# selbouhaddani/PPLS

Measured on AMD Instinct MI355X. Metric: EM iterations/sec + log-lik rel-err vs CPU ref, n=1e6 p=q=2000 r=5, higher is better.
Workload: dtype f64

## Files before the change

### include/ppls_debug.h

```cpp
#ifndef PPLS_AMD_PPLS_DEBUG_H
#define PPLS_AMD_PPLS_DEBUG_H

#include "ppls.h"

#ifdef __cplusplus
extern "C" {
#endif

int ppls_sweep_timing(ppls_ctx* ctx, double* total_ms, int64_t* launches, int reset);
int ppls_sweep_balance(ppls_ctx* ctx, double* w8, int64_t* bounds, int cap, int* n_bounds);
int ppls_comm_info(ppls_ctx* ctx, int* nranks, int* rank, double* allreduce_ms, int64_t* allreduce_calls,
                   int reset);
int ppls_xprod_info(ppls_ctx* ctx, int r, int* ready, int64_t* bytes_per_pass, double* flops, int* rows_per_wave);
int ppls_xprod_setup_times(ppls_ctx* ctx, double* gram_ms, double* allreduce_ms, double* total_ms);
int ppls_xprod_tile_timing(ppls_ctx* ctx, int reps, double* ms);
int ppls_xprod_stats(ppls_ctx* ctx, const ppls_theta* th, int r, double* stats);
int ppls_sweep_stats(ppls_ctx* ctx, const ppls_theta* th, int r, int want_mu, double* stats, double* mu);
int ppls_finalize_stats(ppls_ctx* ctx, const ppls_theta* th, int r, int type, int iter, const double* stats,
                        const double* gram_cur, const double* vstate_in, const double* xpM, int ldx, int ldy,
                        double* W_next, double* C_next, double* scalars, ppls_expect* mom, double* loglik,
                        double* gram_nxt, double* vstate_out, double* gram_stats, int* status3);
int ppls_finalize_plan(ppls_ctx* ctx, int r, int type, int* templated, int* KX, int* KY, int* staged,
                       int64_t* stage_budget);
int ppls_sweep_info(ppls_ctx* ctx, int r, int64_t* bytes_per_sweep, int* variant, int* grid);
int ppls_sweep_kernel(ppls_ctx* ctx, int r, char* buf, int len);
int ppls_gram_int8(ppls_ctx* ctx, int which, double* G, int* nmod, int* L, double* ms);
int ppls_gram_shifts(ppls_ctx* ctx, int* shift, int P, int* count);
int ppls_oz_residue_host(double x, int shift, int l, int* r);
int ppls_oz_crt_host(const int* r, int nmod, double* out);
int ppls_oz_modulus(int l);
int ppls_gram_info(ppls_ctx* ctx, int* int8_used, int* nmod, int* L, double* ms);
int ppls_meta_info(ppls_ctx* ctx, int* path);
int ppls_meta_xprod_info(ppls_ctx* ctx, int* npop, int64_t* formations, double* form_ms);
int ppls_xprod_meta_stats(ppls_ctx* ctx, const double* W, const double* C, const double* params, double* stats);
int ppls_xprod_meta_timing(ppls_ctx* ctx, int reps, double* ms);
int ppls_xprod_meta_nt(int K, int P);
int ppls_rank1_mu_coefficients(const double* params5, double* coef4);
int ppls_gram(ppls_ctx* ctx, int xory, int nsplit, double* G, double* ms);
int ppls_gram_weighted(ppls_ctx* ctx, int xory, int nsplit, const int32_t* count, double* G, double* ms);
int ppls_xgram_permuted(ppls_ctx* ctx, int nsplit, const int64_t* perm, double* C , double* ms);
int ppls_xperm_occupancy(int f32);
int ppls_xperm_timing(ppls_ctx* ctx, double* ms4);
int ppls_gram_occupancy(int f32);
int ppls_gram_occupancy_weighted(int f32);
int ppls_spd_inverse(ppls_ctx* ctx, const double* A, int p, int a, int method, double* out, int* info, double* ms);
int ppls_philox4x32_10(ppls_ctx* ctx, const uint32_t* ctr, int64_t count, uint64_t key, uint32_t* out);

#define PPLS_FTRACE_LEN 48
int ppls_finalize_trace(ppls_ctx* ctx, int64_t* stamps, double* tick_ns);
#define PPLS_STRACE_MAX_WG 4096
int ppls_sweep_trace(ppls_ctx* ctx, int64_t* stamps, int cap, int* n, double* tick_ns);
int ppls_cv_timing(ppls_ctx* ctx, double* out6, int reset);

int ppls_xprod_get(ppls_ctx* ctx, double* S, int* P, int* ldx);
// ... 20 lines not shown
```

### ppls_amd/_lib.py

```python
from __future__ import annotations

import ctypes as ct
import os

import numpy as np

_HERE = os.path.dirname(os.path.abspath(__file__))
LIB_PATH = os.path.join(_HERE, "libppls_amd.so")

PPLS_OK = 0
PPLS_ORTH_SVD = 0
PPLS_ORTH_QR = 1
PPLS_LAYOUT_COLMAJOR = 0
PPLS_LAYOUT_ROWMAJOR = 1

_dp = ct.POINTER(ct.c_double)


class PplsTheta(ct.Structure):
    _fields_ = [("W", _dp), ("C", _dp), ("B", _dp), ("sigT", _dp),
                ("sigE", ct.c_double), ("sigF", ct.c_double), ("sigH", ct.c_double)]


class PplsExpect(ct.Structure):
# ... 86 lines not shown
    "ppls_finalize_stats": (ct.c_int, [ct.c_void_p, ct.POINTER(PplsTheta), ct.c_int, ct.c_int, ct.c_int, _dp, _dp, _dp,
                                       _dp, ct.c_int, ct.c_int, _dp, _dp, _dp, ct.POINTER(PplsExpect), _dp, _dp,
                                       _dp, _dp, ct.POINTER(ct.c_int)]),
    "ppls_finalize_plan": (ct.c_int, [ct.c_void_p, ct.c_int, ct.c_int, ct.POINTER(ct.c_int), ct.POINTER(ct.c_int),
                                      ct.POINTER(ct.c_int), ct.POINTER(ct.c_int), ct.POINTER(ct.c_int64)]),
    "ppls_xprod_info": (ct.c_int, [ct.c_void_p, ct.c_int, ct.POINTER(ct.c_int), ct.POINTER(ct.c_int64), _dp,
                                   ct.POINTER(ct.c_int)]),
    "ppls_sweep_timing": (ct.c_int, [ct.c_void_p, _dp, ct.POINTER(ct.c_int64), ct.c_int]),
    "ppls_sweep_balance": (ct.c_int, [ct.c_void_p, _dp, ct.POINTER(ct.c_int64), ct.c_int, ct.POINTER(ct.c_int)]),
    "ppls_comm_info": (ct.c_int, [ct.c_void_p, ct.POINTER(ct.c_int), ct.POINTER(ct.c_int), _dp,
                                  ct.POINTER(ct.c_int64), ct.c_int]),
    "ppls_finalize_trace": (ct.c_int, [ct.c_void_p, ct.POINTER(ct.c_int64), _dp]),
    "ppls_sweep_trace": (ct.c_int, [ct.c_void_p, ct.POINTER(ct.c_int64), ct.c_int, ct.POINTER(ct.c_int), _dp]),
    "ppls_sweep_info": (ct.c_int, [ct.c_void_p, ct.c_int, ct.POINTER(ct.c_int64), ct.POINTER(ct.c_int),
                                   ct.POINTER(ct.c_int)]),
    "ppls_sweep_kernel": (ct.c_int, [ct.c_void_p, ct.c_int, ct.c_char_p, ct.c_int]),
    "ppls_meta_info": (ct.c_int, [ct.c_void_p, ct.POINTER(ct.c_int)]),
    "ppls_gram_int8": (ct.c_int, [ct.c_void_p, ct.c_int, _dp, ct.POINTER(ct.c_int), ct.POINTER(ct.c_int), _dp]),
    "ppls_oz_residue_host": (ct.c_int, [ct.c_double, ct.c_int, ct.c_int, ct.POINTER(ct.c_int)]),
    "ppls_oz_crt_host": (ct.c_int, [ct.POINTER(ct.c_int), ct.c_int, _dp]),
    "ppls_oz_modulus": (ct.c_int, [ct.c_int]),
    "ppls_gram_info": (ct.c_int, [ct.c_void_p, ct.POINTER(ct.c_int), ct.POINTER(ct.c_int), ct.POINTER(ct.c_int),
                                  _dp]),
    "ppls_gram_shifts": (ct.c_int, [ct.c_void_p, ct.POINTER(ct.c_int), ct.c_int, ct.POINTER(ct.c_int)]),
    "ppls_finalize_host": (ct.c_int, [_dp, _dp, _dp, ct.c_double, ct.c_double, ct.c_double, ct.c_int,
                                      ct.c_int, ct.c_int, ct.POINTER(PplsTheta), ct.c_int,
                                      ct.POINTER(PplsTheta), ct.POINTER(PplsExpect), _dp]),
    "ppls_mu_coefficients": (ct.c_int, [ct.POINTER(PplsTheta), ct.c_int, _dp]),
    "ppls_set_data_from": (ct.c_int, [ct.c_void_p, ct.c_void_p, _i64p, ct.c_int64, ct.c_int64]),
    "ppls_xprod_downdate": (ct.c_int, [ct.c_void_p, ct.c_void_p, _i64p, ct.c_int64]),
    "ppls_xprod_resample": (ct.c_int, [ct.c_void_p, ct.c_void_p, ct.POINTER(ct.c_int32)]),
    "ppls_xprod_permute": (ct.c_int, [ct.c_void_p, ct.c_void_p, _i64p]),
    "ppls_xgram_permuted": (ct.c_int, [ct.c_void_p, ct.c_int, _i64p, _dp, _dp]),
    "ppls_xperm_occupancy": (ct.c_int, [ct.c_int]),
    "ppls_xperm_timing": (ct.c_int, [ct.c_void_p, _dp]),
    "ppls_predict": (ct.c_int, [ct.c_void_p, _dp, _dp, _dp, ct.c_int, ct.c_int, _dp, ct.c_int64, ct.c_int, _dp]),
    "ppls_heldout_sse": (ct.c_int, [ct.c_void_p, _dp, _dp, _dp, ct.c_int, _i64p, ct.c_int64, _dp]),
    "ppls_cv_ppls": (ct.c_int, [ct.c_void_p, ct.c_int, ct.c_int, ct.POINTER(ct.c_int32), _i64p, ct.c_int,
                                ct.c_double, ct.c_int, ct.POINTER(PplsTheta), _dp, ct.POINTER(ct.c_int)]),
    "ppls_cv_timing": (ct.c_int, [ct.c_void_p, _dp, ct.c_int]),
    "ppls_scale_data": (ct.c_int, [ct.c_void_p, ct.c_int, ct.c_int]),
    "ppls_get_scaling": (ct.c_int, [ct.c_void_p, _dp, _dp]),
    "ppls_scale_timing": (ct.c_int, [ct.c_void_p, _dp, _dp]),
    "ppls_xprod_get": (ct.c_int, [ct.c_void_p, _dp, ct.POINTER(ct.c_int), ct.POINTER(ct.c_int)]),
    "ppls_stream_begin":(ct.c_int, [ct.c_void_p, ct.c_int, ct.c_int, ct.c_int, ct.c_int]),
    "ppls_stream_rows": (ct.c_int, [ct.c_void_p, _dp, _dp, ct.c_int64, ct.c_int]),
# ... 131 lines not shown
```

### ppls_amd/api.py

```python
from __future__ import annotations

import ctypes as ct
import itertools
import math
import time
import warnings

import numpy as np

from . import _lib
from ._lib import Expect, PplsError, Theta, dptr


def pop_rows(pop_sizes, row0, n_local):
    sizes = np.asarray(pop_sizes, dtype=np.int64)
    ends = np.cumsum(sizes)
    begins = ends - sizes
    lo, hi = int(row0), int(row0) + int(n_local)
    local = np.clip(np.minimum(ends, hi) - np.maximum(begins, lo), 0, None).astype(np.int64)
    return np.ascontiguousarray(local), np.ascontiguousarray(sizes)


class Context:

# ... 529 lines not shown
        return G, ms.value

    def gram_occupancy(self, f32=False, weighted=False):
        fn = self._L.ppls_gram_occupancy_weighted if weighted else self._L.ppls_gram_occupancy
        return int(fn(int(bool(f32))))

    def gram_int8(self, which=2, want=True):
        P = self.p if which == 0 else self.q if which == 1 else int(round(np.sqrt(self.xprod_info()["bytes_per_pass"] / 8)))
        G = np.zeros((P, P), order="F") if want else None
        nm, L, ms = ct.c_int(), ct.c_int(), np.zeros(4)
        self._chk(self._L.ppls_gram_int8(self.h, int(which), dptr(G), ct.byref(nm), ct.byref(L), dptr(ms)))
        return G, dict(nmod=nm.value, L=L.value, ms=ms.tolist(), shift=self.gram_shifts())

    def gram_shifts(self):
        k = ct.c_int()
        self._chk(self._L.ppls_gram_shifts(self.h, None, 0, ct.byref(k)))
        out = (ct.c_int * max(k.value, 1))()
        self._chk(self._L.ppls_gram_shifts(self.h, out, k.value, ct.byref(k)))
        return np.array(out[:k.value], dtype=np.int64)

    def gram_info(self):
        u, nm, L, ms = ct.c_int(), ct.c_int(), ct.c_int(), np.zeros(4)
        self._chk(self._L.ppls_gram_info(self.h, ct.byref(u), ct.byref(nm), ct.byref(L), dptr(ms)))
        return dict(int8=bool(u.value), nmod=nm.value, L=L.value, ms=ms.tolist())

    def spd_inverse(self, A, method=1):
        A = np.asarray(A, dtype=np.float64)
        one = A.ndim == 2
        A3 = A[None] if one else A
        a, p = A3.shape[0], A3.shape[1]
        Af = np.ascontiguousarray(np.transpose(A3, (0, 2, 1)))
        out = np.empty_like(Af)
        info = (ct.c_int * a)()
        ms = ct.c_double()
        self._chk(self._L.ppls_spd_inverse(self.h, dptr(Af), int(p), int(a), int(method), dptr(out), info,
                                            ct.byref(ms)))
        inv = np.transpose(out, (0, 2, 1))
        return (inv[0] if one else inv), np.array(list(info)), ms.value

    def xprod_prepare(self):
        ms, tot = ct.c_double(), ct.c_double()
        self._chk(self._L.ppls_xprod_prepare(self.h, ct.byref(ms), ct.byref(tot)))
        return ms.value, tot.value

    def xprod_release(self):
        self._chk(self._L.ppls_xprod_release(self.h))
        self._stream_folds = None
# ... 1384 lines not shown
```

### ppls_amd/csrc/ppls_capi.cpp

```cpp
#include <hip/hip_runtime.h>
#include <rccl/rccl.h>
#include <rocblas/rocblas.h>
#include <rocsolver/rocsolver.h>

#include <algorithm>
#include <atomic>
#include <chrono>
#include <cmath>
#include <cstdarg>
#include <cstdio>
#include <cstring>
#include <functional>
#include <string>
#include <utility>
#include <vector>

#include "../../include/ppls.h"
#include "../../include/ppls_debug.h"
#include "ppls_kernels.h"
#include "ppls_math.h"
#include "ppls_cv.h"
#include "ppls_o2m.h"
#include "ppls_permute.h"
#include "ppls_scale.h"
// ... 59 lines not shown
  int* status = nullptr;
  long long* ftrace = nullptr;
  unsigned* team_bar = nullptr;
  double* team_part = nullptr;
  long long* strace = nullptr;
  int balance = 0;
  bool bal_done = false;
  int64_t bal_n = -1;
  int bal_grid = -1;
  double bal_w[8] = {1, 1, 1, 1, 1, 1, 1, 1};
  int64_t* bal_bounds = nullptr;
  double* coefs = nullptr;
  double* scratch = nullptr;
  size_t scratch_bytes = 0;
  int* stop_d = nullptr;
  int* stop_mirror = nullptr;
  int* stop_mirror_dev = nullptr;
  const int* sweep_stop = nullptr;
  double stop_atol = 0.0;
  int em_r = 0, em_cur = 0, em_iter = 0;
  bool em_active = false;
  int xprod = 0;
  int xprod_rw = 0;
  int gram_int8 = 0;
  int oz_used = 0, oz_nmod = 0, oz_L = 0;
  std::vector<int> oz_shift;
  double oz_ms[4] = {0, 0, 0, 0};
  int8_t* oz_planes = nullptr;
  uint8_t* oz_res = nullptr;
  size_t oz_planes_len = 0, oz_res_len = 0;
  bool xp_ready = false;
  bool xp_active = false;
  bool xp_pending_gram = false;
  int xprod_fuse = 1;
  bool xp_explicit = false;
  int meta_path = 0;
  int meta_xprod = 0;
  double* mx_S = nullptr;
  int mx_K = 0;
  std::vector<int64_t> mx_local, mx_total;
  int64_t mx_formations = 0;
  double mx_form_ms = 0.0;
  int meta_device = 1;
  int vorth = 8;
  double* xp_S = nullptr;
  double* xp_M = nullptr;
  double xp_setup_ms = 0.0;
  double xp_setup_total_ms = 0.0;
  double xp_setup_ar_ms = 0.0;
  int xp_nsplit = 0;
  int* gram_q = nullptr;
  int64_t gq_key[8] = {-1, -1, -1, -1, -1, -1, -1, -1};
  rocblas_handle blas = nullptr;
// ... 81 lines not shown
    if (e_ != hipSuccess)                                                                 \
      return fail((c), PPLS_E_HIP, "%s: %s (%s:%d)", #call, hipGetErrorString(e_), __FILE__, \
                  __LINE__);                                                              \
  } while (0)

#define RCCLCHK(c, call)                                                                  \
  do {                                                                                    \
    ncclResult_t e_ = (call);                                                             \
    if (e_ != ncclSuccess)                                                                \
      return fail((c), PPLS_E_COMM, "%s: %s", #call, ncclGetErrorString(e_));            \
  } while (0)

void oz_free(ppls_ctx* c);
bool oz_held(const ppls_ctx* c);

template <typename T>
int dalloc(ppls_ctx* c, T** p, size_t count) {
  if (*p) {
    (void)hipFree(*p);
    *p = nullptr;
  }
  if (count == 0) count = 1;
  hipError_t e = hipMalloc((void**)p, count * sizeof(T));
  if (e == hipErrorOutOfMemory && oz_held(c) && (void*)p != (void*)&c->oz_planes && (void*)p != (void*)&c->oz_res) {
    (void)hipGetLastError();
    (void)hipStreamSynchronize(c->stream);
    oz_free(c);
    e = hipMalloc((void**)p, count * sizeof(T));
  }
  if (e != hipSuccess) {
    *p = nullptr;
    return fail(c, PPLS_E_NOMEM, "hipMalloc(%zu bytes): %s", count * sizeof(T), hipGetErrorString(e));
  }
  return PPLS_OK;
}

template <typename T>
void dfree(T*& p) {
  if (p) (void)hipFree(p);
  p = nullptr;
}

int ld_of(int p, int f32 = 0, int pad = 1) {
  const int es = f32 ? 4 : 8;
  const long bytes = (long)p * es;
  if (!pad || bytes < 1024 || (!f32 && p <= 2048)) return f32 ? (p + 3) & ~3 : (p + 1) & ~1;
  const long al = bytes >= 16384 ? 4096 : 128;
// ... 494 lines not shown
  if (!part_in && (rc = dalloc(c, &part, (size_t)ppls_gram_part_doubles(g.p, nsplit)))) return rc;
  if ((rc = gram_queue(c, g, n, req, &q))) { if (!part_in) dfree(part); return rc; }
  hipEvent_t e0 = nullptr, e1 = nullptr;
  hipError_t e = hipSuccess;
  if (ms) {
    e = hipEventCreate(&e0);
    if (e == hipSuccess) e = hipEventCreate(&e1);
    if (e == hipSuccess) e = hipEventRecord(e0, c->stream);
  }
  if (e == hipSuccess)
    e = ppls_launch_gram_joint(g.X, g.ldx, g.xcols, g.xreal, g.Y, g.ldy, g.ycols, g.yreal, c->dtype, n, g.p, nsplit, part,
                               q, cnt, c->stream);
  if (e == hipSuccess && ms) e = hipEventRecord(e1, c->stream);
  if (e == hipSuccess) e = ppls_launch_gram_finish(part, nsplit, g.p, g.xreal, g.xcols, g.yreal, G, c->stream);
  if (e == hipSuccess) e = hipStreamSynchronize(c->stream);
  if (e == hipSuccess && ms) e = hipEventElapsedTime(ms, e0, e1);
  if (e0) (void)hipEventDestroy(e0);
  if (e1) (void)hipEventDestroy(e1);
  if (!part_in) dfree(part);
  if (e != hipSuccess) return fail(c, PPLS_E_HIP, "MFMA Gram: %s", hipGetErrorString(e));
  return PPLS_OK;
}

bool oz_held(const ppls_ctx* c) { return c->oz_planes || c->oz_res; }

void oz_free(ppls_ctx* c) {
  dfree(c->oz_planes);
  dfree(c->oz_res);
  c->oz_planes = nullptr;
  c->oz_res = nullptr;
  c->oz_planes_len = c->oz_res_len = 0;
}

int gram_run_oz(ppls_ctx* c, const GramShape& g, int64_t n, double* G, float* ms) {
  const int P = g.p, Pp = (P + 255) / 256 * 256;
  const int64_t nkb = (n + PPLS_OZ_KS - 1) / PPLS_OZ_KS;
  const int dtype = c->dtype;
  struct Bufs {
    double* part = nullptr;
    double* st = nullptr;
    int* shift = nullptr;
    hipEvent_t ev[5] = {nullptr, nullptr, nullptr, nullptr, nullptr};
    ~Bufs() {
      dfree(part); dfree(st); dfree(shift);
      for (auto e : ev) if (e) (void)hipEventDestroy(e);
    }
  } b;
  int rc;
  const int chunks = (int)std::max<int64_t>(1, std::min<int64_t>(256, n / 2048));
  if ((rc = dalloc(c, &b.part, (size_t)chunks * 2 * Pp)) || (rc = dalloc(c, &b.st, (size_t)2 * Pp)) ||
      (rc = dalloc(c, &b.shift, (size_t)Pp)))
    return rc;
  for (auto& e : b.ev) HIPCHK(c, hipEventCreate(&e));
  HIPCHK(c, hipEventRecord(b.ev[0], c->stream));
// ... 8 lines not shown
  double qmax = 0.0;
  for (int j = 0; j < P; ++j) {
    if (!live(j) || !(st[(size_t)j] > 0.0)) continue;
    int ex = 0;
    (void)std::frexp(st[(size_t)j], &ex);
    const double cj = std::max(1.0, std::ldexp(1.0, ex) * std::sqrt((double)n / st[(size_t)Pp + j]));
    const int Lj = 53 + (int)std::ceil(std::log2(cj)) + 2;
    L = std::max(L, Lj);
    shift[(size_t)j] = Lj - ex;
    const double q = std::ldexp(std::sqrt(st[(size_t)Pp + j]), Lj - ex) + 0.5 * std::sqrt((double)n);
    qmax = std::max(qmax, q * q);
  }
  c->oz_L = L;
  c->oz_shift.assign(shift.begin(), shift.begin() + P);
  if (L > 62) return 1;
  const double need = std::log2(std::max(qmax, 1.0)) + 1.0 + 1e-7;
  double bits = 0.0;
  int nmod = 0;
  while (nmod < PPLS_OZ_MAXMOD && bits < need) bits += std::log2((double)ppls_oz_modulus(nmod++));
  if (bits < need) return 1;
  nmod = std::max(nmod, 12);
  c->oz_nmod = nmod;
  const int T = Pp / 256, ntiles = T * (T + 1) / 2, nsplit = ppls_oz_splits(nkb);
  const int64_t pstride = nkb * Pp * PPLS_OZ_KS;
  const size_t need_planes = (size_t)nmod * pstride, need_res = (size_t)nmod * nsplit * ntiles * 65536;
  if (need_planes > c->oz_planes_len || need_res > c->oz_res_len) {
    HIPCHK(c, hipStreamSynchronize(c->stream));
    oz_free(c);
    size_t fr = 0, tot = 0;
    if (hipMemGetInfo(&fr, &tot) != hipSuccess) return 1;
    const double want = (double)need_planes + (double)need_res;
    if (want > (double)fr - std::max(1073741824.0, 0.05 * (double)fr)) return 1;
    if (dalloc(c, &c->oz_planes, need_planes) || dalloc(c, &c->oz_res, need_res)) {
      c->err.clear();
      oz_free(c);
      return 1;
    }
    c->oz_planes_len = need_planes;
    c->oz_res_len = need_res;
  }
  int8_t* planes = c->oz_planes;
  uint8_t* res = c->oz_res;
  HIPCHK(c, hipMemcpyAsync(b.shift, shift.data(), sizeof(int) * Pp, hipMemcpyHostToDevice, c->stream));
  HIPCHK(c, ppls_launch_oz_residues(g.X, g.ldx, g.xcols, g.xreal, g.Y, g.ldy, g.yreal, dtype, Pp, n, nkb, b.shift,
                                    nmod, planes, pstride, c->stream));
  HIPCHK(c, hipEventRecord(b.ev[1], c->stream));
  HIPCHK(c, ppls_launch_oz_syrk(planes, pstride, Pp, nkb, nmod, res, c->stream));
  HIPCHK(c, hipEventRecord(b.ev[2], c->stream));
  HIPCHK(c, ppls_launch_oz_finish(res, nmod, nsplit, Pp, g.xcols, g.xreal, g.yreal, P, b.shift, G, c->stream));
  HIPCHK(c, hipEventRecord(b.ev[3], c->stream));
  HIPCHK(c, hipStreamSynchronize(c->stream));
  float t01 = 0.f, t12 = 0.f, t23 = 0.f, t03 = 0.f;
  HIPCHK(c, hipEventElapsedTime(&t01, b.ev[0], b.ev[1]));
  HIPCHK(c, hipEventElapsedTime(&t12, b.ev[1], b.ev[2]));
  HIPCHK(c, hipEventElapsedTime(&t23, b.ev[2], b.ev[3]));
  HIPCHK(c, hipEventElapsedTime(&t03, b.ev[0], b.ev[3]));
  c->oz_ms[0] = t01;
  c->oz_ms[1] = t12;
  c->oz_ms[2] = t23;
  c->oz_ms[3] = t03;
  if (ms) *ms = t03;
  return PPLS_OK;
}

int gram_run_s(ppls_ctx* c, const GramShape& g, int64_t n, double* G, float* ms, double* part) {
  c->oz_used = 0;
  if (c->gram_int8) {
    const int rc = gram_run_oz(c, g, n, G, ms);
    if (rc == PPLS_OK) {
      c->oz_used = 1;
      return PPLS_OK;
    }
    if (rc < 0) return rc;
  }
  return gram_run(c, g, n, 0, G, ms, part);
}

int xprod_setup(ppls_ctx* c);
bool xprod_choose(ppls_ctx* c, int max_steps, int r);

int64_t xprod_rows(const ppls_ctx* c) { return (c->n_total + c->nranks - 1) / c->nranks; }

double xprod_bytes(ppls_ctx* c) {
  const GramShape g = gram_shape(c, true, 0);
  const double PP = (double)g.p * g.p;
  return 8.0 * PP + 8.0 * (double)ppls_gram_part_doubles(g.p, gram_nsplit(c, g, xprod_rows(c), 0)) +
         16.0 * g.p * PPLS_RMAX;
}

int xprod_begin(ppls_ctx* c, int steps, int r) {
// ... 49 lines not shown
  }
  const auto ta = std::chrono::steady_clock::now();
  if ((rc = allreduce(c, c->xp_S, PP))) return rc;
  HIPCHK(c, hipStreamSynchronize(c->stream));
  c->xp_setup_ar_ms = collective(c) ? std::chrono::duration<double, std::milli>(std::chrono::steady_clock::now() - ta).count() : 0.0;
  c->xp_setup_total_ms = std::chrono::duration<double, std::milli>(std::chrono::steady_clock::now() - t0).count();
  c->xp_ready = true;
  c->xp_serial = ++g_xp_serial;
  return PPLS_OK;
}

bool xprod_choose(ppls_ctx* c, int max_steps, int r) {
  if (c->st_state == 2) return true;
  if (c->xprod == 0) return false;
  if (c->xprod == 1) return true;
  if (!c->xp_ready && xprod_bytes(c) > c->mem_free_min - std::max(1073741824.0, 0.05 * c->mem_free_min))
    return false;
  const double P = (double)(c->ldx + c->ldy);
  const double n = (double)((c->n_total + c->nranks - 1) / c->nranks);
  const double esz = c->dtype ? 4.0 : 8.0;
  const bool split = c->sweep_mode != 3 && !c->dtype && ppls_split_supported(r, c->ldx, c->ldy) > 0;
  const double t_sweep = (split ? 1.0 : 2.0) * esz * n * P / 6.5e12 + 5e-6;
  const double t_pass = 8.0 * P * P / 6.5e12 + 5e-6;
  const double gram_rate = c->gram_int8 ? 1.0e14 : 55e12;
  const double t_setup = c->xp_ready ? 0.0 : n * P * P / gram_rate + (c->nranks > 1 ? 16.0 * P * P / 100e9 : 0.0);
  return ((double)max_steps + 1.0) * (t_sweep - t_pass) > t_setup;
}

int xprod_stats(ppls_ctx* c, int r, int slot, bool fuse) {
  int rc;
  const int P = c->ldx + c->ldy;
  if (!c->xp_ready && (rc = xprod_setup(c))) return rc;
  if (!c->xp_M) {
    if ((rc = dalloc(c, &c->xp_M, (size_t)P * 2 * PPLS_RMAX))) return rc;
  }
  hipEvent_t e0, e1;
  if ((rc = timing_pair(c, &e0, &e1))) return rc;
  if (e0) HIPCHK(c, hipEventRecord(e0, c->stream));
  const int rw = ppls_xprod_tile_rows(P, r, c->xprod_rw, c->num_cus);
  const bool defer = fuse && c->xprod_fuse && r <= 8 && P <= 6144;
  HIPCHK(c, ppls_launch_xprod_tile(c->xp_S, c->ldx, c->ldy, r, rw, c->W[slot], c->C[slot], c->sc[slot], c->stats,
                                   c->xp_M, c->sweep_stop, defer ? 0 : 1, c->stream));
  c->xp_pending_gram = defer;
  if (e1) HIPCHK(c, hipEventRecord(e1, c->stream));
  return PPLS_OK;
}

// ... 407 lines not shown
    c->xprod = (int)value;
    if (value == 0 && was != 0 && !c->xp_explicit && c->st_state == 0) {
      HIPCHK(c, hipStreamSynchronize(c->stream));
      xprod_free(c);
    }
  } else if (!strcmp(key, "meta_device")) {
    c->meta_device = value ? 1 : 0;
  } else if (!strcmp(key, "meta_xprod")) {
    if (value != 0 && value != 1) return fail(c, PPLS_E_ARG, "meta_xprod must be 0 (sweep the rows) or 1 (population cross-products)");
    c->meta_xprod = (int)value;
    if (!c->meta_xprod && c->mx_S) {
      HIPCHK(c, hipStreamSynchronize(c->stream));
      meta_xp_free(c);
    }
  } else if (!strcmp(key, "vorth")) {
    if (value < 1 || value > 255) return fail(c, PPLS_E_ARG, "vorth must be in [1, 255]");
    c->vorth = (int)value;
  } else if (!strcmp(key, "xprod_fuse")) {
    c->xprod_fuse = value ? 1 : 0;
  } else if (!strcmp(key, "var_chol")) {
    if (value < 0 || value > 2) return fail(c, PPLS_E_ARG, "var_chol must be 0 (LU), 1 (Cholesky) or 2 (rocSOLVER Cholesky)");
    c->var_chol = (int)value;
  } else if (!strcmp(key, "gram_int8")) {
    if (value < 0 || value > 1) return fail(c, PPLS_E_ARG, "gram_int8 must be 0 (fp64 MFMA Gram) or 1 (int8 CRT form)");
    if ((int)value != c->gram_int8) {
      c->gram_int8 = (int)value;
      if (c->xp_ready && !c->xp_explicit) {
        dfree(c->xp_S);
        c->xp_ready = false;
      }
      if (!c->gram_int8) {
        HIPCHK(c, hipStreamSynchronize(c->stream));
        oz_free(c);
      }
    }
  } else if (!strcmp(key, "xprod_rw")) {
    if (value != 0 && value != 1 && value != 2 && value != 4 && value != 8)
      return fail(c, PPLS_E_ARG, "xprod_rw must be 0, 1, 2, 4 or 8");
    c->xprod_rw = (int)value;
  } else if (!strcmp(key, "o2m_path")) {
    if (value < 0 || value > 2) return fail(c, PPLS_E_ARG, "o2m_path must be 0 (auto), 1 (fused) or 2 (two-phase)");
    c->o2m_path = (int)value;
  } else if (!strcmp(key, "timing")) {
    if (value < 0) return fail(c, PPLS_E_ARG, "timing must be >= 0");
    c->timing = (int)value;
    c->sweep_count = 0;
  } else {
    return fail(c, PPLS_E_ARG, "unknown option '%s'", key);
  }
  return PPLS_OK;
}

void ppls_shard_range(int64_t n_total, int nranks, int rank, int64_t* row0, int64_t* n_local) {
  if (nranks < 1) nranks = 1;
  const int64_t b = n_total * rank / nranks, e = n_total * (rank + 1) / nranks;
  if (row0) *row0 = b;
  if (n_local) *n_local = e - b;
}
// ... 2849 lines not shown
    rc = fail(c, PPLS_E_HIP, "int8 gram: copy-out failed");
  dfree(dG);
  if (!rc && ms) for (int k = 0; k < 4; ++k) ms[k] = c->oz_ms[k];
  return rc;
}

int ppls_gram_shifts(ppls_ctx* c, int* shift, int P, int* count) {
  if (!c) return PPLS_E_ARG;
  const int k = (int)c->oz_shift.size();
  if (count) *count = k;
  if (shift) for (int j = 0; j < std::min(P, k); ++j) shift[j] = c->oz_shift[(size_t)j];
  return PPLS_OK;
}

int ppls_gram_info(ppls_ctx* c, int* int8_used, int* nmod, int* L, double* ms) {
  if (!c) return PPLS_E_ARG;
  if (int8_used) *int8_used = c->oz_used;
  if (nmod) *nmod = c->oz_nmod;
  if (L) *L = c->oz_L;
  if (ms) for (int k = 0; k < 4; ++k) ms[k] = c->oz_ms[k];
  return PPLS_OK;
}

int ppls_meta_info(ppls_ctx* c, int* path) {
  if (!c || !path) return PPLS_E_ARG;
  *path = c->meta_path;
  return PPLS_OK;
}

int ppls_sweep_kernel(ppls_ctx* c, int r, char* buf, int len) {
  if (!c || !buf || len < 1) return PPLS_E_ARG;
  if (r < 1 || r > PPLS_RMAX) return fail(c, PPLS_E_ARG, "bad r");
  PplsSweepArgs a;
  const int plan = sweep_plan(c, r, &a);
  const int nt = c->nt_loads > 0 ||
                 (c->nt_loads < 0 && 8.0 * sweep_rows(c) * (double)(c->ldx + c->ldy) > 256.0 * (1 << 20));
  char k[128];
  if (plan == 3) {
    if (ppls_split_describe(&a, k, sizeof k) != 0) return fail(c, PPLS_E_STATE, "no split instantiation for r=%d", r);
  } else {
    const bool rows64 = c->dots_rows ? c->dots_rows == 64 : sweep_rows(c) >= 32768;
    const int64_t wtiles = (sweep_rows(c) + (rows64 ? 63 : 31)) / (rows64 ? 64 : 32);
    const bool pair = c->dots_pair >= 0 ? c->dots_pair == 1 : wtiles < (int64_t)c->num_cus * 4 * (rows64 ? 2 : 3);
    snprintf(k, sizeof k, "panel<%s,%d> (mfmadots %d rows/%s + acc, %d chunks)", c->dtype ? "float" : "double", r,
             rows64 ? 64 : 32, pair ? "wave pair" : "wave", a.grid);
  }
// ... 395 lines not shown
  std::vector<std::vector<int64_t>> in_fold((size_t)nfolds);
  for (int64_t i = 0; i < c->n_local; ++i) {
    if (fold_of_row[i] < 0 || fold_of_row[i] >= nfolds) return fail(c, PPLS_E_ARG, "fold_of_row[%lld]=%d outside [0,%d)", (long long)i, fold_of_row[i], nfolds);
    in_fold[(size_t)fold_of_row[i]].push_back(i);
  }
  for (int f = 0; f < nfolds; ++f)
    if ((int64_t)in_fold[(size_t)f].size() > fold_total[f])
      return fail(c, PPLS_E_ARG, "fold %d: %zu local rows, %lld over all ranks", f, in_fold[(size_t)f].size(), (long long)fold_total[f]);
  for (int k = 0; !o2m && k < nfolds * a; ++k)
    if (!init[k].W || !init[k].C || !init[k].B || !init[k].sigT) return fail(c, PPLS_E_ARG, "init[%d] has NULL fields", k);
  HIPCHK(c, hipSetDevice(c->device));
  int rc;
  if (!c->cv_train && (rc = ppls_ctx_create(c->device, &c->cv_train))) return fail(c, rc, "could not create the training context");
  ppls_ctx* t = c->cv_train;
  t->xprod = c->xprod;
  t->xprod_rw = c->xprod_rw;
  t->xprod_fuse = c->xprod_fuse;
  t->o2m_path = c->o2m_path;
  if (t->gram_int8 && !c->gram_int8) {
    HIPCHK(c, hipStreamSynchronize(t->stream));
    oz_free(t);
  }
  t->gram_int8 = c->gram_int8;
  t->ldpad = c->ldpad;
  t->sweep_mode = c->sweep_mode;
  t->grid_opt = c->grid_opt;
  t->nt_loads = c->nt_loads;
  t->reducer = c->reducer;
  t->reducer_user = c->reducer_user;
  t->comm = c->comm;
  t->nranks = c->nranks;
  t->rank = c->rank;
  const int p = c->p, q = c->q;
  std::vector<double> W((size_t)p * a), C((size_t)q * a), B((size_t)a), sig((size_t)4 * a), sse((size_t)a);
  std::vector<int64_t> train;
  for (int f = 0; f < nfolds; ++f) {
    const std::vector<int64_t>& out = in_fold[(size_t)f];
    train.clear();
    for (int64_t i = 0; i < c->n_local; ++i)
      if (fold_of_row[i] != f) train.push_back(i);
    const int64_t n_train = c->n_total - fold_total[f];
    if (n_train < 1) return fail(c, PPLS_E_ARG, "fold %d leaves no training row", f);
    if ((rc = ppls_set_data_from(t, c, train.data(), (int64_t)train.size(), n_train))) { c->err = t->err; return rc; }
    if ((o2m || xprod_choose(t, a * max_steps, 1)) && fold_total[f] <= n_train)
      if ((rc = ppls_xprod_downdate(t, c, out.data(), (int64_t)out.size()))) { c->err = t->err; return rc; }
    ppls_seq_fit fit;
// ... 1455 lines not shown
```

### ppls_amd/csrc/ppls_kernels.h

```cpp
#pragma once

#include <hip/hip_runtime.h>
#include <stdint.h>

#include "ppls_math.h"

#define PPLS_SWEEP_SLOTS 4
#define PPLS_FUSED_RMAX 8

struct PplsSweepArgs {
  const double* X;
  const double* Y;
  int64_t n_local;
  int p, q;
  int ldx, ldy;
  const double* Wp;
  const double* Cp;
  const PplsScalars* sc;
  double* part;
  int64_t part_ld;
  double* mu;
  int write_mu;
  int r;
  int ns;
// ... 70 lines not shown
  const double* Cp;
  int m;
  PplsRank1* st;
  double* tw;
  double* tc;
  const double* consW;
  const double* consC;
  PplsRank1 cons_val;
  int cons_mask;
  double* Wdst;
  double* Cdst;
  PplsScalars* scdst;
  double* lv;
  double* Gkeep;
  int step, max_steps, crit_abs;
  double atol;
  int* stop;
  int* stop_mirror;
};

#define PPLS_META_KMAX 1024
#define PPLS_OZ_MAXMOD 20
#define PPLS_OZ_KS 64
struct PplsMetaStepArgs {
  const double* stats;
  int64_t part_ld;
  int K, p, q, ldx, ldy;
  const double* N;
  const double* ssq;
  PplsRank1* st;
  PplsScalars* sc;
  double* W;
  double* C;
  double* log;
  int64_t log_ld;
  int step, max_steps, crit_abs;
  double atol;
  int* stop;
  int* stop_mirror;
  double ssqX, ssqY, Ntot;
};

extern "C" {
hipError_t ppls_launch_meta_step(const PplsMetaStepArgs* a, hipStream_t st);
int ppls_split_supported(int r, int ldx, int ldy);
hipError_t ppls_launch_sweep_split(const PplsSweepArgs* a, hipStream_t st);
// ... 43 lines not shown
hipError_t ppls_launch_xtmu(const void* X, int f32, int64_t n, int ld, const double* mu, int a, int chunks,
                            double* part, int64_t part_ld, hipStream_t st);
hipError_t ppls_launch_varmat(const double* G, const double* cxt, const double* w, int p, double ctt, double k1,
                              double k2, double bstar, double s4, double N, double* M, double* sst_exp,
                              double* sst_star, hipStream_t st);
hipError_t ppls_launch_negdiag(double* M, int p, double* se, hipStream_t st);
hipError_t ppls_launch_negate(double* M, int64_t len, hipStream_t st);
hipError_t ppls_launch_symdiag(double* M, int p, double* se, hipStream_t st);
int64_t ppls_spd_inverse_work(int p, int a);
hipError_t ppls_spd_inverse_batched(double* A, int p, int a, double* work, int* info, hipStream_t st);
hipError_t ppls_launch_to_colmajor(const double* src, int64_t n, int p, int ld, double* dst,
                                   hipStream_t st);
int ppls_oz_modulus(int l);
hipError_t ppls_launch_oz_colstats(const void* X, int ldx, int xcols, int xreal, const void* Y, int ldy, int yreal,
                                   int f32, int Pp, int64_t n, int chunks, double* part, double* out, hipStream_t st);
hipError_t ppls_launch_oz_residues(const void* X, int ldx, int xcols, int xreal, const void* Y, int ldy, int yreal,
                                   int f32, int Pp, int64_t n, int64_t nkb, const int* shift, int nmod, int8_t* planes,
                                   int64_t pstride, hipStream_t st);
int ppls_oz_splits(int64_t nkb);
hipError_t ppls_launch_oz_syrk(const int8_t* planes, int64_t pstride, int Pp, int64_t nkb, int nmod, uint8_t* part,
                               hipStream_t st);
hipError_t ppls_launch_oz_finish(const uint8_t* part, int nmod, int nsplit, int Pp, int xcols, int xreal, int yreal,
                                 int P, const int* shift, double* G, hipStream_t st);
}
```

### ppls_amd/csrc/ppls_ozaki.hip

```cpp
#include <hip/hip_runtime.h>
#include <stdint.h>

#include <type_traits>

#include "ppls_device.h"
#include "ppls_kernels.h"

namespace {

constexpr int OZ_TT = 256;
constexpr int OZ_KS = PPLS_OZ_KS;
constexpr int OZ_PANEL = OZ_TT * OZ_KS;
constexpr int OZ_SPLIT_STAGES = 1024;

__host__ __device__ constexpr int oz_mod(int l) {
  switch (l) {
    case 0: return 256;  case 1: return 255;  case 2: return 253;  case 3: return 251;  case 4: return 247;
    case 5: return 241;  case 6: return 239;  case 7: return 233;  case 8: return 229;  case 9: return 227;
    case 10: return 223; case 11: return 217; case 12: return 211; case 13: return 199; case 14: return 197;
    case 15: return 193; case 16: return 191; case 17: return 181; case 18: return 179; case 19: return 173;
    default: return 1;
  }
}

// ... 244 lines not shown
    for (int j = 0; j < NJ; ++j)
#pragma unroll
      for (int r = 0; r < 16; ++r) {
        const int v = acc[i][j][r] % m;
        acc[i][j][r] = v < 0 ? v + m : v;
      }
  if (idle) return;
  uint8_t* o = out + (int64_t)it * OZ_TT * OZ_TT;
#pragma unroll
  for (int i = 0; i < 4; ++i)
#pragma unroll
    for (int j = 0; j < NJ; ++j) {
      const int col = CT * wj + 32 * j + (lane & 31);
#pragma unroll
      for (int gq = 0; gq < 4; ++gq) {
        const int row = 128 * wi + 32 * i + 8 * gq + 4 * h;
        const uint32_t v = (uint32_t)acc[i][j][4 * gq] | ((uint32_t)acc[i][j][4 * gq + 1] << 8) |
                           ((uint32_t)acc[i][j][4 * gq + 2] << 16) | ((uint32_t)acc[i][j][4 * gq + 3] << 24);
        *(uint32_t*)(o + (int64_t)col * OZ_TT + row) = v;
      }
    }
}

namespace {

template <int NMOD>
__host__ __device__ __forceinline__ double oz_crt(const int (&r)[NMOD], const OzTab& tab) {
  int d[NMOD];
#pragma unroll
  for (int l = 0; l < NMOD; ++l) {
    const int m = oz_mod(l);
    int t = r[l];
#pragma unroll
    for (int k = 0; k < l; ++k) {
      t = t - d[k] + 2 * m;
      t = (t * tab.inv[l][k]) % m;
    }
    d[l] = t;
  }
  uint32_t v[6] = {(uint32_t)d[NMOD - 1], 0, 0, 0, 0, 0};
#pragma unroll
  for (int l = NMOD - 2; l >= 0; --l) {
    uint64_t carry = (uint64_t)d[l];
#pragma unroll
    for (int q = 0; q < 6; ++q) {
      const uint64_t x = (uint64_t)v[q] * (uint64_t)oz_mod(l) + carry;
// ... 162 lines not shown
  const int64_t grid = (items + 7) / 8 * 8;
  if (grid > 0x7fffffff) return hipErrorInvalidValue;
#define OZ_SYRK(AV)                                                                                             \
  case AV:                                                                                                      \
    hipLaunchKernelGGL(ppls_oz_syrk_kernel<AV>, dim3((unsigned)grid), dim3(((AV) & 4) ? 512 : 256), 0, st, planes, \
                       pstride, Pp, nkb, nmod, nsplit, ntiles, part);                                           \
    break;
  switch (variant) {
    OZ_SYRK(0)
#ifdef OZ_LAB
    OZ_SYRK(1) OZ_SYRK(2) OZ_SYRK(4) OZ_SYRK(5) OZ_SYRK(6)
#endif
    default: return hipErrorInvalidValue;
  }
#undef OZ_SYRK
  return hipGetLastError();
}

hipError_t ppls_launch_oz_syrk(const int8_t* planes, int64_t pstride, int Pp, int64_t nkb, int nmod, uint8_t* part,
                               hipStream_t st) {
  return ppls_launch_oz_syrk_v(0, planes, pstride, Pp, nkb, nmod, part, st);
}

hipError_t ppls_launch_oz_finish(const uint8_t* part, int nmod, int nsplit, int Pp, int xcols, int xreal, int yreal,
                                 int P, const int* shift, double* G, hipStream_t st) {
  const OzCols g{xreal, xcols, yreal};
  const int T = Pp / OZ_TT, ntiles = T * (T + 1) / 2;
  const dim3 grid((unsigned)ntiles, (unsigned)(OZ_TT / 16));
#define OZ_FIN(N)                                                                                               \
  case N:                                                                                                       \
    hipLaunchKernelGGL((ppls_oz_finish_kernel<N>), grid, dim3(256), 0, st, part, nsplit, ntiles, g, P, shift, G); \
    break;
  switch (nmod) {
    OZ_NMOD_CASES(OZ_FIN)
    default: return hipErrorInvalidValue;
  }
#undef OZ_FIN
  return hipGetLastError();
}

}
```

Baseline: 207.9.

## Auto-enable int8 Ozaki Gram by size and process rows in bounded groups

The int8 CRT (Ozaki) Gram path now defaults to an auto mode that switches on when rows·P² is large, which covers this workload's size. The single large residue-plane and partial-result buffers are replaced by one workspace sized by a planner. The planner splits the rows into groups that fit a fraction of HBM, runs residues and syrk per group, and folds partial residues modulo each prime into an accumulator before the final CRT. This is meant to replace the fp64 MFMA Gram with integer matrix ops while bounding memory, at the cost of an extra fold kernel per group and a per-call memory query. The change of default also alters the cost model that decides whether the cross-product path is used.

```diff
diff --git a/include/ppls_debug.h b/include/ppls_debug.h
--- a/include/ppls_debug.h
+++ b/include/ppls_debug.h
@@ -30,6 +30,10 @@
 int ppls_oz_crt_host(const int* r, int nmod, double* out);
 int ppls_oz_modulus(int l);
 int ppls_gram_info(ppls_ctx* ctx, int* int8_used, int* nmod, int* L, double* ms);
+int64_t ppls_oz_plan_groups(int64_t n, int Pp, int nmod, int num_cus, int64_t total_hbm, int64_t free_hbm,
+                            int force_group, int* G);
+int ppls_gram_int8_plan(ppls_ctx* ctx, int* group, int64_t* ws_bytes);
+int ppls_gram_int8_auto(int64_t n_total, int nranks, int P);
 int ppls_meta_info(ppls_ctx* ctx, int* path);
 int ppls_meta_xprod_info(ppls_ctx* ctx, int* npop, int64_t* formations, double* form_ms);
 int ppls_xprod_meta_stats(ppls_ctx* ctx, const double* W, const double* C, const double* params, double* stats);
diff --git a/ppls_amd/_lib.py b/ppls_amd/_lib.py
--- a/ppls_amd/_lib.py
+++ b/ppls_amd/_lib.py
@@ -132,6 +132,10 @@
     "ppls_oz_modulus": (ct.c_int, [ct.c_int]),
     "ppls_gram_info": (ct.c_int, [ct.c_void_p, ct.POINTER(ct.c_int), ct.POINTER(ct.c_int), ct.POINTER(ct.c_int),
                                   _dp]),
+    "ppls_oz_plan_groups": (ct.c_int64, [ct.c_int64, ct.c_int, ct.c_int, ct.c_int, ct.c_int64, ct.c_int64, ct.c_int,
+                                         ct.POINTER(ct.c_int)]),
+    "ppls_gram_int8_plan": (ct.c_int, [ct.c_void_p, ct.POINTER(ct.c_int), ct.POINTER(ct.c_int64)]),
+    "ppls_gram_int8_auto": (ct.c_int, [ct.c_int64, ct.c_int, ct.c_int]),
     "ppls_gram_shifts": (ct.c_int, [ct.c_void_p, ct.POINTER(ct.c_int), ct.c_int, ct.POINTER(ct.c_int)]),
     "ppls_finalize_host": (ct.c_int, [_dp, _dp, _dp, ct.c_double, ct.c_double, ct.c_double, ct.c_int,
                                       ct.c_int, ct.c_int, ct.POINTER(PplsTheta), ct.c_int,
diff --git a/ppls_amd/api.py b/ppls_amd/api.py
--- a/ppls_amd/api.py
+++ b/ppls_amd/api.py
@@ -575,7 +575,9 @@
     def gram_info(self):
         u, nm, L, ms = ct.c_int(), ct.c_int(), ct.c_int(), np.zeros(4)
         self._chk(self._L.ppls_gram_info(self.h, ct.byref(u), ct.byref(nm), ct.byref(L), dptr(ms)))
-        return dict(int8=bool(u.value), nmod=nm.value, L=L.value, ms=ms.tolist())
+        G, ws = ct.c_int(), ct.c_int64()
+        self._chk(self._L.ppls_gram_int8_plan(self.h, ct.byref(G), ct.byref(ws)))
+        return dict(int8=bool(u.value), nmod=nm.value, L=L.value, ms=ms.tolist(), group=G.value, ws_bytes=ws.value)
 
     def spd_inverse(self, A, method=1):
         A = np.asarray(A, dtype=np.float64)
diff --git a/ppls_amd/csrc/ppls_capi.cpp b/ppls_amd/csrc/ppls_capi.cpp
--- a/ppls_amd/csrc/ppls_capi.cpp
+++ b/ppls_amd/csrc/ppls_capi.cpp
@@ -105,13 +105,14 @@
   bool em_active = false;
   int xprod = 0;
   int xprod_rw = 0;
-  int gram_int8 = 0;
+  int gram_int8 = -1;
+  int oz_group = 0;
   int oz_used = 0, oz_nmod = 0, oz_L = 0;
+  int oz_G = 0;
   std::vector<int> oz_shift;
   double oz_ms[4] = {0, 0, 0, 0};
-  int8_t* oz_planes = nullptr;
-  uint8_t* oz_res = nullptr;
-  size_t oz_planes_len = 0, oz_res_len = 0;
+  uint8_t* oz_ws = nullptr;
+  size_t oz_ws_len = 0;
   bool xp_ready = false;
   bool xp_active = false;
   bool xp_pending_gram = false;
@@ -239,7 +240,7 @@
   }
   if (count == 0) count = 1;
   hipError_t e = hipMalloc((void**)p, count * sizeof(T));
-  if (e == hipErrorOutOfMemory && oz_held(c) && (void*)p != (void*)&c->oz_planes && (void*)p != (void*)&c->oz_res) {
+  if (e == hipErrorOutOfMemory && oz_held(c) && (void*)p != (void*)&c->oz_ws) {
     (void)hipGetLastError();
     (void)hipStreamSynchronize(c->stream);
     oz_free(c);
@@ -780,14 +781,15 @@
   return PPLS_OK;
 }
 
-bool oz_held(const ppls_ctx* c) { return c->oz_planes || c->oz_res; }
+bool oz_held(const ppls_ctx* c) { return c->oz_ws != nullptr; }
 
 void oz_free(ppls_ctx* c) {
-  dfree(c->oz_planes);
-  dfree(c->oz_res);
-  c->oz_planes = nullptr;
-  c->oz_res = nullptr;
-  c->oz_planes_len = c->oz_res_len = 0;
+  dfree(c->oz_ws);
+  c->oz_ws_len = 0;
+}
+
+bool gram_wants_int8(const ppls_ctx* c, int P) {
+  return c->gram_int8 == 1 || (c->gram_int8 < 0 && ppls_gram_int8_auto(c->n_total, c->nranks, P));
 }
 
 int gram_run_oz(ppls_ctx* c, const GramShape& g, int64_t n, double* G, float* ms) {
@@ -842,41 +844,67 @@
   nmod = std::max(nmod, 12);
   c->oz_nmod = nmod;
   const int T = Pp / 256, ntiles = T * (T + 1) / 2, nsplit = ppls_oz_splits(nkb);
-  const int64_t pstride = nkb * Pp * PPLS_OZ_KS;
-  const size_t need_planes = (size_t)nmod * pstride, need_res = (size_t)nmod * nsplit * ntiles * 65536;
-  if (need_planes > c->oz_planes_len || need_res > c->oz_res_len) {
+  size_t fr = 0, tot = 0;
+  if (hipMemGetInfo(&fr, &tot) != hipSuccess) return 1;
+  int Gs = 0;
+  const int64_t ws_need = ppls_oz_plan_groups(n, Pp, nmod, c->num_cus, (int64_t)tot, (int64_t)(fr + c->oz_ws_len),
+                                           c->oz_group, &Gs);
+  if (ws_need <= 0) return 1;
+  if ((size_t)ws_need > c->oz_ws_len) {
     HIPCHK(c, hipStreamSynchronize(c->stream));
     oz_free(c);
-    size_t fr = 0, tot = 0;
-    if (hipMemGetInfo(&fr, &tot) != hipSuccess) return 1;
-    const double want = (double)need_planes + (double)need_res;
-    if (want > (double)fr - std::max(1073741824.0, 0.05 * (double)fr)) return 1;
-    if (dalloc(c, &c->oz_planes, need_planes) || dalloc(c, &c->oz_res, need_res)) {
+    if (dalloc(c, &c->oz_ws, (size_t)ws_need)) {
       c->err.clear();
       oz_free(c);
       return 1;
     }
-    c->oz_planes_len = need_planes;
-    c->oz_res_len = need_res;
-  }
-  int8_t* planes = c->oz_planes;
-  uint8_t* res = c->oz_res;
+    c->oz_ws_len = (size_t)ws_need;
+  }
+  c->oz_G = Gs;
+  const int ngroups = (nsplit + Gs - 1) / Gs;
+  const int64_t gstages = std::min<int64_t>((int64_t)Gs * 1024, nkb), grows = (int64_t)Gs * 65536;
+  const size_t plane_bytes = (size_t)nmod * gstages * Pp * PPLS_OZ_KS;
+  int8_t* planes = (int8_t*)c->oz_ws;
+  uint8_t* res = c->oz_ws + plane_bytes;
+  uint8_t* acc = res + (size_t)nmod * Gs * ntiles * 65536;
+  struct GroupEvents {
+    std::vector<hipEvent_t> v;
+    ~GroupEvents() { for (auto e : v) if (e) (void)hipEventDestroy(e); }
+  } ge;
+  ge.v.assign((size_t)2 * ngroups, nullptr);
+  for (auto& e : ge.v) HIPCHK(c, hipEventCreate(&e));
   HIPCHK(c, hipMemcpyAsync(b.shift, shift.data(), sizeof(int) * Pp, hipMemcpyHostToDevice, c->stream));
-  HIPCHK(c, ppls_launch_oz_residues(g.X, g.ldx, g.xcols, g.xreal, g.Y, g.ldy, g.yreal, dtype, Pp, n, nkb, b.shift,
-                                    nmod, planes, pstride, c->stream));
-  HIPCHK(c, hipEventRecord(b.ev[1], c->stream));
-  HIPCHK(c, ppls_launch_oz_syrk(planes, pstride, Pp, nkb, nmod, res, c->stream));
+  const size_t esz = dtype ? 4 : 8;
+  for (int k = 0; k < ngroups; ++k) {
+    const int64_t row0 = (int64_t)k * grows, rows = std::min<int64_t>(grows, n - row0);
+    const int64_t nkb_k = (rows + PPLS_OZ_KS - 1) / PPLS_OZ_KS, pstride = nkb_k * Pp * PPLS_OZ_KS;
+    const void* Xk = (const char*)g.X + (size_t)row0 * g.ldx * esz;
+    const void* Yk = g.Y ? (const void*)((const char*)g.Y + (size_t)row0 * g.ldy * esz) : nullptr;
+    HIPCHK(c, ppls_launch_oz_residues(Xk, g.ldx, g.xcols, g.xreal, Yk, g.ldy, g.yreal, dtype, Pp, rows, nkb_k, b.shift,
+                                      nmod, planes, pstride, c->stream));
+    HIPCHK(c, hipEventRecord(ge.v[(size_t)2 * k], c->stream));
+    HIPCHK(c, ppls_launch_oz_syrk(planes, pstride, Pp, nkb_k, nmod, res, c->stream));
+    HIPCHK(c, hipEventRecord(ge.v[(size_t)2 * k + 1], c->stream));
+    if (ngroups > 1) HIPCHK(c, ppls_launch_oz_fold(res, nmod, ppls_oz_splits(nkb_k), Pp, acc, k == 0, c->stream));
+  }
   HIPCHK(c, hipEventRecord(b.ev[2], c->stream));
-  HIPCHK(c, ppls_launch_oz_finish(res, nmod, nsplit, Pp, g.xcols, g.xreal, g.yreal, P, b.shift, G, c->stream));
+  if (ngroups > 1)
+    HIPCHK(c, ppls_launch_oz_finish(acc, nmod, 1, Pp, g.xcols, g.xreal, g.yreal, P, b.shift, G, c->stream));
+  else
+    HIPCHK(c, ppls_launch_oz_finish(res, nmod, nsplit, Pp, g.xcols, g.xreal, g.yreal, P, b.shift, G, c->stream));
   HIPCHK(c, hipEventRecord(b.ev[3], c->stream));
   HIPCHK(c, hipStreamSynchronize(c->stream));
-  float t01 = 0.f, t12 = 0.f, t23 = 0.f, t03 = 0.f;
-  HIPCHK(c, hipEventElapsedTime(&t01, b.ev[0], b.ev[1]));
-  HIPCHK(c, hipEventElapsedTime(&t12, b.ev[1], b.ev[2]));
+  float t23 = 0.f, t03 = 0.f;
+  double tsyrk = 0.0;
+  for (int k = 0; k < ngroups; ++k) {
+    float t = 0.f;
+    HIPCHK(c, hipEventElapsedTime(&t, ge.v[(size_t)2 * k], ge.v[(size_t)2 * k + 1]));
+    tsyrk += t;
+  }
   HIPCHK(c, hipEventElapsedTime(&t23, b.ev[2], b.ev[3]));
   HIPCHK(c, hipEventElapsedTime(&t03, b.ev[0], b.ev[3]));
-  c->oz_ms[0] = t01;
-  c->oz_ms[1] = t12;
+  c->oz_ms[0] = std::max(0.0, (double)t03 - tsyrk - (double)t23);
+  c->oz_ms[1] = tsyrk;
   c->oz_ms[2] = t23;
   c->oz_ms[3] = t03;
   if (ms) *ms = t03;
@@ -885,7 +913,7 @@
 
 int gram_run_s(ppls_ctx* c, const GramShape& g, int64_t n, double* G, float* ms, double* part) {
   c->oz_used = 0;
-  if (c->gram_int8) {
+  if (gram_wants_int8(c, g.p)) {
     const int rc = gram_run_oz(c, g, n, G, ms);
     if (rc == PPLS_OK) {
       c->oz_used = 1;
@@ -981,7 +1009,7 @@
   const bool split = c->sweep_mode != 3 && !c->dtype && ppls_split_supported(r, c->ldx, c->ldy) > 0;
   const double t_sweep = (split ? 1.0 : 2.0) * esz * n * P / 6.5e12 + 5e-6;
   const double t_pass = 8.0 * P * P / 6.5e12 + 5e-6;
-  const double gram_rate = c->gram_int8 ? 1.0e14 : 55e12;
+  const double gram_rate = gram_wants_int8(c, c->ldx + c->ldy) ? 1.0e14 : 55e12;
   const double t_setup = c->xp_ready ? 0.0 : n * P * P / gram_rate + (c->nranks > 1 ? 16.0 * P * P / 100e9 : 0.0);
   return ((double)max_steps + 1.0) * (t_sweep - t_pass) > t_setup;
 }
@@ -1435,7 +1463,8 @@
     if (value < 0 || value > 2) return fail(c, PPLS_E_ARG, "var_chol must be 0 (LU), 1 (Cholesky) or 2 (rocSOLVER Cholesky)");
     c->var_chol = (int)value;
   } else if (!strcmp(key, "gram_int8")) {
-    if (value < 0 || value > 1) return fail(c, PPLS_E_ARG, "gram_int8 must be 0 (fp64 MFMA Gram) or 1 (int8 CRT form)");
+    if (value < -1 || value > 1)
+      return fail(c, PPLS_E_ARG, "gram_int8 must be -1 (auto: by size), 0 (fp64 MFMA Gram) or 1 (int8 CRT form)");
     if ((int)value != c->gram_int8) {
       c->gram_int8 = (int)value;
       if (c->xp_ready && !c->xp_explicit) {
@@ -1447,6 +1476,9 @@
         oz_free(c);
       }
     }
+  } else if (!strcmp(key, "oz_group")) {
+    if (value < 0 || value > 0x7fffffff) return fail(c, PPLS_E_ARG, "oz_group must be 0 (auto) or the splits per row group");
+    c->oz_group = (int)value;
   } else if (!strcmp(key, "xprod_rw")) {
     if (value != 0 && value != 1 && value != 2 && value != 4 && value != 8)
       return fail(c, PPLS_E_ARG, "xprod_rw must be 0, 1, 2, 4 or 8");
@@ -4342,6 +4374,13 @@
   return PPLS_OK;
 }
 
+int ppls_gram_int8_plan(ppls_ctx* c, int* group, int64_t* ws_bytes) {
+  if (!c) return PPLS_E_ARG;
+  if (group) *group = c->oz_G;
+  if (ws_bytes) *ws_bytes = (int64_t)c->oz_ws_len;
+  return PPLS_OK;
+}
+
 int ppls_meta_info(ppls_ctx* c, int* path) {
   if (!c || !path) return PPLS_E_ARG;
   *path = c->meta_path;
@@ -4783,6 +4822,7 @@
     oz_free(t);
   }
   t->gram_int8 = c->gram_int8;
+  t->oz_group = c->oz_group;
   t->ldpad = c->ldpad;
   t->sweep_mode = c->sweep_mode;
   t->grid_opt = c->grid_opt;
diff --git a/ppls_amd/csrc/ppls_kernels.h b/ppls_amd/csrc/ppls_kernels.h
--- a/ppls_amd/csrc/ppls_kernels.h
+++ b/ppls_amd/csrc/ppls_kernels.h
@@ -116,6 +116,7 @@
 #define PPLS_META_KMAX 1024
 #define PPLS_OZ_MAXMOD 20
 #define PPLS_OZ_KS 64
+#define PPLS_OZ_AUTO_NPP 4e12
 struct PplsMetaStepArgs {
   const double* stats;
   int64_t part_ld;
@@ -205,4 +206,8 @@
                                hipStream_t st);
 hipError_t ppls_launch_oz_finish(const uint8_t* part, int nmod, int nsplit, int Pp, int xcols, int xreal, int yreal,
                                  int P, const int* shift, double* G, hipStream_t st);
+hipError_t ppls_launch_oz_fold(const uint8_t* grp, int nmod, int G, int Pp, uint8_t* acc, int first, hipStream_t st);
+int64_t ppls_oz_plan_groups(int64_t n, int Pp, int nmod, int num_cus, int64_t total_hbm, int64_t free_hbm,
+                            int force_group, int* G);
+int ppls_gram_int8_auto(int64_t n_total, int nranks, int P);
 }
diff --git a/ppls_amd/csrc/ppls_ozaki.hip b/ppls_amd/csrc/ppls_ozaki.hip
--- a/ppls_amd/csrc/ppls_ozaki.hip
+++ b/ppls_amd/csrc/ppls_ozaki.hip
@@ -290,6 +290,31 @@
     }
 }
 
+__global__ __launch_bounds__(256) void ppls_oz_fold_kernel(const uint8_t* __restrict__ grp, int G, int ntiles,
+                                                           uint8_t* __restrict__ acc, int first) {
+  const int l = blockIdx.y;
+  const int64_t i = (int64_t)blockIdx.x * 256 + threadIdx.x;
+  if (i >= (int64_t)ntiles * (OZ_TT * OZ_TT / 16)) return;
+  const uint32_t m = (uint32_t)oz_mod(l);
+  const int64_t t = i / (OZ_TT * OZ_TT / 16), off = (i % (OZ_TT * OZ_TT / 16)) * 16;
+  uint8_t* a = acc + ((int64_t)l * ntiles + t) * OZ_TT * OZ_TT + off;
+  v4i s = first ? v4i{0, 0, 0, 0} : *(const v4i*)a;
+  for (int sp = 0; sp < G; ++sp) {
+    const v4i x = *(const v4i*)(grp + (((int64_t)l * G + sp) * ntiles + t) * OZ_TT * OZ_TT + off);
+#pragma unroll
+    for (int w = 0; w < 4; ++w) {
+      uint32_t o = 0;
+#pragma unroll
+      for (int b = 0; b < 4; ++b) {
+        const uint32_t v = (((uint32_t)s[w] >> (8 * b)) & 255u) + (((uint32_t)x[w] >> (8 * b)) & 255u);
+        o |= (v % m) << (8 * b);
+      }
+      s[w] = (int)o;
+    }
+  }
+  *(v4i*)a = s;
+}
+
 namespace {
 
 template <int NMOD>
@@ -498,6 +523,44 @@
   return ppls_launch_oz_syrk_v(0, planes, pstride, Pp, nkb, nmod, part, st);
 }
 
+hipError_t ppls_launch_oz_fold(const uint8_t* grp, int nmod, int G, int Pp, uint8_t* acc, int first, hipStream_t st) {
+  const int T = Pp / OZ_TT, ntiles = T * (T + 1) / 2;
+  const dim3 grid((unsigned)(ntiles * (OZ_TT * OZ_TT / 16 / 256)), (unsigned)nmod);
+  hipLaunchKernelGGL(ppls_oz_fold_kernel, grid, dim3(256), 0, st, grp, G, ntiles, acc, first);
+  return hipGetLastError();
+}
+
+int64_t ppls_oz_plan_groups(int64_t n, int Pp, int nmod, int num_cus, int64_t total_hbm, int64_t free_hbm,
+                            int force_group, int* G) {
+  if (n < 1 || Pp < OZ_TT || Pp % OZ_TT || nmod < 1 || num_cus < 1) return 0;
+  const int64_t nkb = (n + OZ_KS - 1) / OZ_KS;
+  const int64_t nsplit = (nkb + OZ_SPLIT_STAGES - 1) / OZ_SPLIT_STAGES;
+  const int64_t T = Pp / OZ_TT, ntiles = T * (T + 1) / 2, tile = (int64_t)OZ_TT * OZ_TT;
+  const double gate = (double)free_hbm - (1073741824.0 > 0.05 * (double)free_hbm ? 1073741824.0 : 0.05 * (double)free_hbm);
+  const double cap = force_group > 0 ? gate : ((double)total_hbm / 10.0 < gate ? (double)total_hbm / 10.0 : gate);
+  auto bytes = [&](int64_t g) {
+    const int64_t stages = g * OZ_SPLIT_STAGES < nkb ? g * OZ_SPLIT_STAGES : nkb;
+    return nmod * stages * Pp * OZ_KS + nmod * g * ntiles * tile + (g < nsplit ? nmod * ntiles * tile : 0);
+  };
+  int64_t g = force_group > 0 ? force_group : (16 * (int64_t)num_cus + nmod * ntiles - 1) / (nmod * ntiles);
+  g = g < 1 ? 1 : g > nsplit ? nsplit : g;
+  if (g > 63) g = 63;
+  for (;;) {
+    if ((double)bytes(g) <= cap) {
+      if (G) *G = (int)g;
+      return bytes(g);
+    }
+    if (force_group > 0 || g == 1) return 0;
+    --g;
+  }
+}
+
+int ppls_gram_int8_auto(int64_t n_total, int nranks, int P) {
+  if (nranks < 1) nranks = 1;
+  const double rows = (double)((n_total + nranks - 1) / nranks);
+  return rows * (double)P * (double)P >= PPLS_OZ_AUTO_NPP ? 1 : 0;
+}
+
 hipError_t ppls_launch_oz_finish(const uint8_t* part, int nmod, int nsplit, int Pp, int xcols, int xreal, int yreal,
                                  int P, const int* shift, double* G, hipStream_t st) {
   const OzCols g{xreal, xcols, yreal};
```

After: 208.0 (median of 5 runs). Within noise of the previous version (+0.1%).
